# AIM-Harvard/pyradiomics

Hardware: AMD Instinct MI355X
Metric: Mvoxels/s for GLCM+GLRLM build, 512^3 vol @32 bins (higher is better)
Workload: dtype u8 levels / u32 counts / f64 out; 1 GPU; GLCM+GLRLM matrix build, 512^3 int32+uint8 volume resident in HBM, 32 grey levels, full mask, 13 angles, uniform levels; one volume per GPU (batch sharding, no collective); size=512, levels=32, dist=uniform, deferred_mode=pipeline

## Files before the change

pyradiomics_amd/csrc/prad_api.hip:

```cpp
#include "prad_runtime.h"
#include "kernels_generic.h"
#include "kernels_pairs.h"
#include "kernels_sweep.h"
#include "kernels_sweepfw.h"
#include "kernels_sweepfw2.h"
#include "kernels_neigh.h"
#include "kernels_glszm.h"
#include "kernels_voxel.h"
#include "kernels_voxslide.h"
#include "kernels_mcc.h"
#include "kernels_voxtex.h"
#include "prad_sweep_plan.h"
#include "prad_internal.h"

#include <algorithm>
#include <atomic>
#include <chrono>
#include <cmath>
#include <condition_variable>
#include <cstdlib>
#include <deque>
#include <limits>
#include <mutex>
#include <thread>
// ... 366 lines not shown
  for (size_t i = (na & ~(size_t)3) + t; i < na; i += nt) a[i] = 0;
  for (size_t i = t; i < nb; i += nt) b[i] = 0;
  for (size_t i = t; i < nc; i += nt) c3[i] = 0;
}

struct VolState {
  bool valid = false;
  SweepPlan p;
  int Ng = 0, Nr = 0, Na = 0;
  double *glcm = nullptr, *glrlm = nullptr;
  uint8_t *levels = nullptr, *rowzero = nullptr;
  uint8_t *levels16 = nullptr;
  u32 *acc = nullptr, *glcm_acc = nullptr, *glrlm_acc = nullptr;
  int *multi = nullptr;
  int *flags_d = nullptr;
  bool packed_inline = false;
  int lane = -1;
};

bool fin_ride(const SweepKnobs &kn) { return kn.fin_ride; }

struct ZeroNeed {
  u32 *acc = nullptr, *rz = nullptr, *fl = nullptr;
  size_t acc_w = 0, rz_w = 0, fl_w = 0;
};
struct SetZero {
  u32 *rz = nullptr, *fl = nullptr;
  size_t rz_cap = 0;
  size_t rz_used = 0;
  size_t rz_zero = 0;
  bool fl_zero = false;
};
constexpr int kPipeSets = 4;
SetZero *set_zero_book() {
  static thread_local SetZero book[kPipeSets];
  return book;
}
void set_zero_forget() {
  for (int i = 0; i < kPipeSets; i++) set_zero_book()[i] = SetZero();
}
int launch_zero3(hipStream_t s, const ZeroNeed &z) {
  const size_t total_w = z.acc_w + z.rz_w + z.fl_w;
  if (total_w == 0) return PRAD_OK;
  const unsigned gx = (unsigned)std::max<size_t>(1, std::min<size_t>((total_w / 4 + 255) / 256, 1024));
  hipLaunchKernelGGL(zero3_kernel, dim3(gx), dim3(256), 0, s, z.acc, z.acc_w, z.rz, z.rz_w, z.fl, z.fl_w);
  return check_launch("zero3_kernel");
}

int vol_prepare(Call &k, const SweepKnobs &kn, const SweepPlan &p, int Ng, int Nr, double *glcm, double *glrlm, VolState &v,
                ZeroNeed *defer = nullptr) {
  Context &c = *k.c;
  v.lane = c.lane;
  v.valid = true;
  v.p = p;
  v.Ng = Ng;
  v.Nr = Nr;
  v.Na = k.Na;
  v.glcm = glcm;
  v.glrlm = glrlm;
  v.flags_d = k.flags_d;
  const long long nrows = (long long)p.Nz * p.Ny;
  v.levels = nullptr;
  if (!(p.fw2 && p.fw2_rows && p.lines.count > 0 && p.row_slot >= 0)) {
    PRAD_TRY(c.get<uint8_t>("levels", (size_t)nrows * p.pitch + 1024, &v.levels));
    v.levels += 512;
  }
  v.levels16 = nullptr;
  if (p.fw2) {
    PRAD_TRY(c.get<uint8_t>("levels16", (size_t)nrows * p.pitch16 + 4096, &v.levels16));
    v.levels16 += 2048;
  }
  const size_t nglcm = glcm ? (size_t)k.Na * Ng * Ng : 0, nglrlm = glrlm ? (size_t)k.Na * Ng * Nr : 0;
  const size_t nctl = 2 * PRAD_MAX_SWEEP + (size_t)PRAD_FW_WORK_STRIDE * (PRAD_FW_DOMAINS * PRAD_MAX_SWEEP + 1);
  PRAD_TRY(c.get<u32>("sweep_acc", nglcm + nglrlm + nctl, &v.acc));
  v.glcm_acc = v.acc;
  v.glrlm_acc = v.acc + nglcm;
  v.multi = (int *)(v.acc + nglcm + nglrlm);
  v.rowzero = nullptr;
  if (p.fw) PRAD_TRY(c.get<uint8_t>("rowzero", (size_t)nrows + 64, &v.rowzero));
  ZeroNeed z;
  z.acc = v.acc;
  z.acc_w = nglcm + nglrlm + nctl;
  z.rz = reinterpret_cast<u32 *>(v.rowzero);
  z.rz_w = v.rowzero ? ((size_t)nrows + 3) / 4 : 0;
  z.fl = reinterpret_cast<u32 *>(v.flags_d);
  z.fl_w = 4;
  if (c.lane >= 0 && c.lane < kPipeSets) {
    SetZero &S = set_zero_book()[c.lane];
    const size_t cap = v.rowzero ? c.bufs[c.key("rowzero")].cap : 0;
    if (fin_ride(kn)) {
      if (S.rz == z.rz && S.rz_cap == cap && z.rz_w <= S.rz_zero) z.rz_w = 0;
      if (S.fl == z.fl && S.fl_zero) z.fl_w = 0;
    }
    S.rz = z.rz;
    S.rz_cap = cap;
    S.rz_used = v.rowzero ? ((size_t)nrows + 3) / 4 : 0;
    S.rz_zero = 0;
    S.fl = z.fl;
    S.fl_zero = false;
  }
  if (defer) {
    *defer = z;
    return PRAD_OK;
  }
  return launch_zero3(k.s, z);
}

bool pipeline_volume(const SweepPlan &p, bool glcm, bool glrlm) {
  if (!(p.ok && p.lines.count > 0 && glcm && glrlm)) return false;
  return (p.fw && p.fused) || p.fw2;
}
bool pack_inline_ok(const Call &k, const VolState &v) {
  if (!(v.glcm && v.glrlm && v.p.pitch == v.p.Nx && v.p.padw == 0 && (k.g.n % 16) == 0 &&
        ((((uintptr_t)k.image) | ((uintptr_t)k.mask) | ((uintptr_t)v.levels)) & 15) == 0))
    return false;
  if (k.g.n >= (1LL << 31)) return false;
  if (v.p.fw2) return v.levels16 && v.p.pitch16 == 2 * v.p.Nx && (((uintptr_t)v.levels16) & 15) == 0;
  return v.p.fw && v.p.fused;
}

// ... 171 lines not shown
      hipLaunchKernelGGL(finalize_glrlm_kernel, dim3(blocks_for((long long)Ng * Nr * Na)), dim3(256), 0, k.s,
                         v.glrlm_acc, v.multi, Ng, Nr, Na, glrlm, (const int *)v.flags_d, sticky);
      PRAD_TRY(check_launch("finalize_glrlm_kernel"));
      latched = sticky != nullptr;
    }
  }
  if (sticky && !latched) {
    hipLaunchKernelGGL(latch_flags_kernel, dim3(1), dim3(1), 0, k.s, v.flags_d, sticky);
    PRAD_TRY(check_launch("latch_flags_kernel"));
  }
  return PRAD_OK;
}

int sweep_glcm_glrlm(Call &k, const SweepKnobs &kn, const SweepPlan &p, int Ng, int Nr, double *glcm, double *glrlm, bool *used) {
  Context &c = *k.c;
  VolState v;
  PRAD_TRY(vol_prepare(k, kn, p, Ng, Nr, glcm, glrlm, v));
  PRAD_TRY(vol_pack_standalone(k, v));
  PackJob pj;
  memset(&pj, 0, sizeof(pj));
  PRAD_TRY(vol_sweep(k, kn, v, pj));
  int *sticky = nullptr;
  if (c.deferred) PRAD_TRY(c.get<int>("deferred_sticky", 16, &sticky));
  PRAD_TRY(vol_finalize(k, kn, v, sticky));
  if (c.deferred) {
    *used = true;
    return PRAD_OK;
  }
  PRAD_TRY(read_flags(k));
  *used = (k.flags_h[0] == 0 && k.flags_h[2] == 0);
  return PRAD_OK;
}

struct PipeState {
  VolState pending;
  VolState walked;
  hipStream_t s = nullptr;
  unsigned long long seq = 0;
  hipEvent_t ev = nullptr;
  int mode = -1;
};
PipeState &pipe_state() {
  static thread_local PipeState p;
  return p;
}
bool pipeline_mode(const SweepKnobs &kn) {
  PipeState &ps = pipe_state();
  if (ps.mode < 0) ps.mode = kn.lanes_mode ? 0 : 1;
  return ps.mode == 1;
}
int pipeline_sticky(Context &c, int **sticky) { return c.get<int>("deferred_sticky", 16, sticky); }

bool fin_job_empty(const FinJob &fj) { return fj.Na == 0 && fj.zn[0] + fj.zn[1] + fj.zn[2] == 0; }

bool fin_can_ride(const SweepKnobs &kn, const VolState &v) {
  const SweepPlan &p = v.p;
  if (!(v.glcm && v.glrlm && p.fw && p.fused && p.lines.count > 0 && v.levels && v.lane >= 0 && v.lane < kPipeSets)) return false;
  if (p.row_slot >= 0 && p.fw_xblocks == 0) return false;
  if (!finalize_one(kn) || (long long)v.Ng * v.Nr >= (1LL << 30) || v.Ng > 255 || v.Na > PRAD_MAX_SWEEP || v.Na != p.aset.count) return false;
  return ((long long)v.Ng * v.Nr + (long long)v.Ng * v.Ng) * v.Na < (1LL << 31);
}
bool fin_host_ok(const SweepKnobs &kn, const PipeState &ps, const VolState &host, const PackJob &pj, hipStream_t s) {
  const SweepPlan &p = host.p;
  if (!(fin_ride(kn) && ps.s == s && host.glcm && host.glrlm && p.fw && p.fused && p.lines.count > 0)) return false;
  const size_t lds = p.fw_xblocks > 0 ? std::max(p.lds_fw, p.lds_fw_rows) : p.lds_fw;
  return lds >= (size_t)PRAD_FIN_SCRATCH_BYTES && p.fw_blocks >= 1 && p.fw_blocks < 32768;
}

FinJob make_fin_job(const VolState &host, const VolState *walked, const ZeroNeed *need, int new_lane) {
  FinJob j;
  memset(&j, 0, sizeof(j));
  const int nline = host.p.fw_blocks;
  if (walked) {
    const VolState &w = *walked;
    j.Na = w.Na;
    j.Ng = w.Ng;
    j.Nr = w.Nr;
    j.Nz = w.p.Nz;
    j.Ny = w.p.Ny;
    j.Nx = w.p.Nx;
    j.pitch = w.p.pitch;
    j.L = w.levels;
    j.glcm_acc = w.glcm_acc;
    j.glrlm_acc = w.glrlm_acc;
    j.glcm_out = w.glcm;
    j.glrlm_out = w.glrlm;
    j.multi = w.multi;
    j.flags = w.flags_d;
    const FwSet &fs = host.p.fwset;
    for (int a = 0; a < w.Na; a++) {
      for (int d = 0; d < 3; d++) j.off[a][d] = (signed char)w.p.aset.off[a][d];
      const int role = a % fs.count, idx = a / fs.count;
      const int b = (fs.first_block[role] + idx < fs.first_block[role + 1]) ? fs.first_block[role] + idx : a % nline;
      j.ablock[a] = (short)b;
    }
  }
  const int wl = walked ? walked->lane : -1;
  if (need && need->acc_w > 0 && new_lane >= 0 && new_lane < kPipeSets && new_lane != host.lane && new_lane != wl) {
    j.z[0] = need->acc;
    j.zn[0] = (unsigned)need->acc_w;
  }
  if (new_lane >= 0 && new_lane < kPipeSets) {
    const int t = (new_lane + 1) % kPipeSets;
    SetZero &S = set_zero_book()[t];
    if (t != host.lane && t != wl && t != new_lane && S.rz_zero < S.rz_used && S.rz) {
      j.z[1] = S.rz;
      j.zn[1] = (unsigned)S.rz_used;
      S.rz_zero = S.rz_used;
    }
    if (t != host.lane && t != wl && t != new_lane && S.fl && !S.fl_zero) {
      j.z[2] = S.fl;
      j.zn[2] = 4;
      S.fl_zero = true;
    }
  }
  return j;
}

int pipeline_finish_walked(Context &c, const SweepKnobs &kn, hipStream_t s) {
  PipeState &ps = pipe_state();
  if (!ps.walked.valid) return PRAD_OK;
  Call k;
  k.c = &c;
  k.s = s;
  k.Na = ps.walked.Na;
  k.flags_d = ps.walked.flags_d;
  int *sticky = nullptr;
  PRAD_TRY(pipeline_sticky(c, &sticky));
  PRAD_TRY(vol_finalize(k, kn, ps.walked, sticky));
  ps.walked.valid = false;
  return PRAD_OK;
}

int pipeline_retire(Context &c, const SweepKnobs &kn, hipStream_t s, const PackJob &pj, bool keep = false, const ZeroNeed *need = nullptr,
                    int new_lane = -1) {
  PipeState &ps = pipe_state();
  const bool host_ok = fin_host_ok(kn, ps, ps.pending, pj, s);
  if (ps.s != s) {
    if (!ps.ev) PRAD_HIP(hipEventCreateWithFlags(&ps.ev, hipEventDisableTiming));
    PRAD_HIP(hipEventRecord(ps.ev, ps.s));
    PRAD_HIP(hipStreamWaitEvent(s, ps.ev, 0));
  }
  Call k;
  k.c = &c;
  k.s = s;
  k.Na = ps.pending.Na;
  k.flags_d = ps.pending.flags_d;
  int *sticky = nullptr;
  PRAD_TRY(pipeline_sticky(c, &sticky));
  FinJob fj;
  memset(&fj, 0, sizeof(fj));
  if (host_ok) {
    const bool rides = ps.walked.valid && fin_can_ride(kn, ps.walked) && ps.walked.lane != ps.pending.lane && ps.walked.lane != new_lane;
    if (ps.walked.valid && !rides) PRAD_TRY(pipeline_finish_walked(c, kn, s));
    fj = make_fin_job(ps.pending, rides ? &ps.walked : nullptr, need, new_lane);
    fj.sticky = sticky;
    ps.walked.valid = false;
  } else {
    PRAD_TRY(pipeline_finish_walked(c, kn, s));
  }
  if (need && need->acc_w > 0 && fj.zn[0] == 0) {
    ZeroNeed acc;
    acc.acc = need->acc;
    acc.acc_w = need->acc_w;
    PRAD_TRY(launch_zero3(s, acc));
  }
  PRAD_TRY(vol_sweep(k, kn, ps.pending, pj, fj));
  if (keep && fin_ride(kn) && fin_can_ride(kn, ps.pending)) {
    ps.walked = ps.pending;
    ps.pending.valid = false;
    return PRAD_OK;
  }
  PRAD_TRY(vol_finalize(k, kn, ps.pending, sticky));
  ps.pending.valid = false;
  return PRAD_OK;
}

int pipeline_flush(Context &c, const SweepKnobs &kn) {
  PipeState &ps = pipe_state();
  if (!ps.pending.valid && !ps.walked.valid) return PRAD_OK;
  PackJob none;
  memset(&none, 0, sizeof(none));
  const size_t before = c.times.size();
  if (ps.pending.valid) PRAD_TRY(pipeline_retire(c, kn, ps.s, none));
  else PRAD_TRY(pipeline_finish_walked(c, kn, ps.s));
  if (c.timing_accumulate) c.all_times.insert(c.all_times.end(), c.times.begin() + (long)before, c.times.end());
  return PRAD_OK;
}
int pipeline_flush(Context &c) {
  PipeState &ps = pipe_state();
  if (!ps.pending.valid && !ps.walked.valid) return PRAD_OK;
  return pipeline_flush(c, sweep_knobs_from_env());
}

int pipeline_step(Call &k, const SweepKnobs &kn, const SweepPlan &p, int Ng, int Nr, double *glcm, double *glrlm, bool *handled) {
  Context &c = *k.c;
  PipeState &ps = pipe_state();
  *handled = false;
  if (!pipeline_volume(p, glcm != nullptr, glrlm != nullptr)) return pipeline_flush(c, kn);
  VolState v;
  ZeroNeed need;
  PRAD_TRY(vol_prepare(k, kn, p, Ng, Nr, glcm, glrlm, v, &need));
  PackJob pj;
  memset(&pj, 0, sizeof(pj));
  bool inl = false;
  if (ps.pending.valid) {
    inl = pack_inline_ok(k, v) && ps.pending.p.fw2 == v.p.fw2 && !kn.no_inline_pack;
    if (inl) pj = make_pack_job(k, kn, v, &ps.pending);
    const bool ride = fin_host_ok(kn, ps, ps.pending, pj, k.s) && need.acc_w + need.rz_w + need.fl_w < ((size_t)1 << 30);
    ZeroNeed now = need;
    if (ride) {
      now.acc_w = 0;
      need.rz_w = need.fl_w = 0;
    }
    PRAD_TRY(launch_zero3(k.s, now));
    PRAD_TRY(pipeline_retire(c, kn, k.s, pj, true, ride ? &need : nullptr, v.lane));
  } else {
    PRAD_TRY(pipeline_finish_walked(c, kn, ps.s));
    PRAD_TRY(launch_zero3(k.s, need));
  }
  if (!inl) PRAD_TRY(vol_pack_standalone(k, v));
  v.packed_inline = inl;
  ps.pending = v;
  ps.s = k.s;
  *handled = true;
  return PRAD_OK;
}

int pairs_glcm_glrlm(Call &k, const SweepKnobs &kn, int Ng, int Nr, double *glcm, double *glrlm, bool *used) {
  *used = false;
  Context &c = *k.c;
  if (k.vm.voxels || k.g.nd > 3 || Ng < 1 || Ng > PRAD_PAIR_LDS_WORDS || k.Na > PRAD_PAIR_MAXA || k.g.n >= 0x7fffffffLL ||
      kn.no_pairs)
    return PRAD_OK;
  int dims[3] = {1, 1, 1};
  for (int d = 0; d < k.g.nd; d++) dims[3 - k.g.nd + d] = k.g.size[d];
  PairAngles A;
  memset(&A, 0, sizeof(A));
  A.n = k.Na;
  for (int a = 0; a < k.Na; a++)
    for (int d = 0; d < k.g.nd; d++) {
      const int o = k.angles_h[a * k.g.nd + d];
      if (o < -127 || o > 127) return PRAD_OK;
      A.o[a][3 - k.g.nd + d] = (signed char)o;
    }
  if (glrlm && Nr < std::max(dims[0], std::max(dims[1], dims[2]))) return PRAD_OK;
  const size_t gwords = glcm ? (size_t)k.Na * Ng * Ng : 0, rwords = glrlm ? (size_t)k.Na * Ng * Nr : 0;
  if ((gwords + rwords) * sizeof(u32) > ((size_t)1 << 30)) return PRAD_OK;
  hipStream_t s = k.s;
  lev16 *L = nullptr;
  u32 *gacc = nullptr, *racc = nullptr, *counts = nullptr;
  int *multi = nullptr;
  PRAD_TRY(c.get<lev16>("pairs_levels", (size_t)k.g.n + 8, &L));
  if (glcm) PRAD_TRY(c.get<u32>("pairs_glcm_acc", gwords, &gacc));
  if (glrlm) {
    PRAD_TRY(c.get<u32>("pairs_glrlm_acc", rwords, &racc));
    PRAD_TRY(c.get<u32>("pairs_counts", (size_t)Ng, &counts));
// ... 57 lines not shown
    PRAD_TRY(check_launch("pairs_glrlm_kernel"));
    hipLaunchKernelGGL(pairs_multi_check_kernel, dim3(gx, (unsigned)k.Na), dim3(256), 0, s, A, L, dims[0], dims[1], dims[2], multi, k.flags_d);
    PRAD_TRY(check_launch("pairs_multi_check_kernel"));
    hipLaunchKernelGGL(pairs_run1_kernel, dim3((unsigned)((Ng * k.Na + 3) / 4)), dim3(256), 0, s, racc, counts, Ng, Nr, k.Na, k.flags_d);
    PRAD_TRY(check_launch("pairs_run1_kernel"));
    const long long total = (long long)Ng * Nr * k.Na;
    hipLaunchKernelGGL(finalize_glrlm_kernel, dim3(blocks_for(total)), dim3(256), 0, s, racc, multi, Ng, Nr, k.Na, glrlm,
                       (const int *)nullptr, (int *)nullptr);
    PRAD_TRY(check_launch("finalize_glrlm_kernel"));
  }
  PRAD_TRY(read_flags(k));
  *used = k.flags_h[0] == 0;
  if (!*used) {
    PRAD_HIP(hipMemsetAsync(k.flags_d, 0, sizeof(int) * 4, s));
  }
  return PRAD_OK;
}

}
namespace prad {
int texture_pairs_runs(const int32_t *image, const uint8_t *mask, const int *size, int Nd, const int *angles,
                       int Na, int Ng, int Nr, int Nvox, const int *voxels, int kernelRadius, int force2Ddim,
                       double *glcm, double *glrlm, hipStream_t s) {
  if (!glcm && !glrlm) return fail(PRAD_E_ARG, "both outputs are NULL");
  if (Ng < 1 || (glrlm && Nr < 1)) return fail(PRAD_E_ARG, "Ng/Nr must be >= 1");
  Context &c = ctx();
  PRAD_TRY(c.ensure_device());
  const SweepKnobs kn = sweep_knobs_from_env();
  struct LaneGuard {
    Context &c;
    ~LaneGuard() { c.lane = -1; }
  } lane_guard{c};
  bool pipe = c.deferred && !voxels && pipeline_mode(kn);
  if (c.deferred && !voxels && !pipe) {
    PRAD_TRY(c.lane_begin(s, &s));
    if (c.lane >= 0) c.lane += kPipeSets;
  }
  if (pipe) c.lane = (int)(pipe_state().seq++ % (unsigned)kPipeSets);
  Call k;
  PRAD_TRY(setup_call(k, image, mask, size, Nd, angles, Na, Nvox, voxels, kernelRadius, force2Ddim, s, false));
  SweepPlan p = plan_sweep(k, kn, Ng, Nr, glcm != nullptr, glrlm != nullptr);
  if (pipe && !pipeline_volume(p, glcm != nullptr, glrlm != nullptr)) {
    const hipStream_t user = s;
    PRAD_TRY(pipeline_flush(c, kn));
    pipe = false;
    c.lane = -1;
    PRAD_TRY(c.lane_begin(user, &s));
    if (c.lane >= 0) c.lane += kPipeSets;
    PRAD_TRY(setup_call(k, image, mask, size, Nd, angles, Na, Nvox, voxels, kernelRadius, force2Ddim, s, false));
    p = plan_sweep(k, kn, Ng, Nr, glcm != nullptr, glrlm != nullptr);
  }
  PRAD_TRY(c.begin_call(s));
  if (!p.ok) PRAD_HIP(hipMemsetAsync(k.flags_d, 0, sizeof(int) * 4, s));
  bool done = false;
  c.last_variant = !p.ok ? "none" : (p.fw2 ? "fw2" : (p.fw && glcm && glrlm ? "fw" : "lines"));
  if (pipe) {
    PRAD_TRY(pipeline_step(k, kn, p, Ng, Nr, glcm, glrlm, &done));
    if (done) c.last_path = "sweep";
  }
  if (!done && p.ok) {
    PRAD_TRY(sweep_glcm_glrlm(k, kn, p, Ng, Nr, glcm, glrlm, &done));
    if (done) c.last_path = "sweep";
  }
  if (!done && !c.deferred) {
    PRAD_TRY(pairs_glcm_glrlm(k, kn, Ng, Nr, glcm, glrlm, &done));
    if (done) {
      c.last_path = "pairs";
      c.last_variant = "pairs";
    }
  }
  if (!done) {
    if (glcm) PRAD_TRY(generic_glcm(k, Ng, glcm));
    if (glrlm) PRAD_TRY(generic_glrlm(k, Ng, Nr, glrlm));
    PRAD_TRY(read_flags(k));
    c.last_path = "generic";
  }
  PRAD_TRY(c.end_call(s));
  if (c.deferred && done) return PRAD_OK;
  PRAD_HIP(hipStreamSynchronize(s));
  return k.flags_h[1] ? PRAD_INDEX_ERROR : PRAD_OK;
}
}
namespace {

int pairs_neigh(Call &k, bool ngtdm, int Ng, int alpha, double *out, bool *used, bool box_only = false) {
  *used = false;
  Context &c = *k.c;
  if (k.vm.voxels || k.g.nd > 3 || Ng < 1 || Ng > 65535 || k.g.n >= 0x7fffffffLL || getenv("PRAD_NO_PAIRS")) return PRAD_OK;
  int dims[3] = {1, 1, 1};
  for (int d = 0; d < k.g.nd; d++) dims[3 - k.g.nd + d] = k.g.size[d];
// ... 460 lines not shown
}

namespace prad {
int zone_features_launch(Context &c, hipStream_t s, const double *P, int Ni, int Njcap, long long stride_i,
                         const double *jvals_d, const int *nj_dev, double *out_d, int *empty_d);
}
extern "C" {

const char *prad_version(void) { return kVersion; }
const char *prad_last_error(void) { return err_state().msg; }
const char *prad_last_path(void) { return ctx().last_path; }
const char *prad_last_variant(void) { return ctx().last_variant; }
#ifdef PRAD_FW_STAMPS
int prad_debug_fw_stamps(unsigned long long *out, int slot, int nwaves) {
  if (!out || nwaves < 1 || nwaves > 8192 || slot < 0 || slot > 1) return PRAD_E_ARG;
  PRAD_HIP(hipDeviceSynchronize());
  PRAD_HIP(hipMemcpyFromSymbol(out, HIP_SYMBOL(prad::prad_fw_stamps), sizeof(unsigned long long) * prad::FP_COUNT * (size_t)nwaves,
                               sizeof(unsigned long long) * prad::FP_COUNT * 8192 * (size_t)slot));
  return PRAD_OK;
}
#endif

int prad_device_count(void) {
  int n = 0;
  if (hipGetDeviceCount(&n) != hipSuccess) return 0;
  return n;
}

int prad_set_device(int device) {
  int n = prad_device_count();
  if (device < 0 || device >= n) return fail(PRAD_E_ARG, "device %d not in [0,%d)", device, n);
  Context &c = ctx();
  if (c.device != device) {
    if ((pipe_state().pending.valid || pipe_state().walked.valid) && c.device_set && hipSetDevice(c.device) == hipSuccess) {
      (void)pipeline_flush(c);
      if (pipe_state().s) (void)hipStreamSynchronize(pipe_state().s);
    }
    pipe_state().pending.valid = false;
    pipe_state().walked.valid = false;
    set_zero_forget();
    pipe_state().s = nullptr;
    pipe_state().ev = nullptr;
    c.own_stream = nullptr;
    for (int l = 0; l < PRAD_MAX_LANES; l++) {
      if (c.lane_stream[l]) (void)hipStreamSynchronize(c.lane_stream[l]);
      c.lane_stream[l] = nullptr;
      c.lane_in[l] = nullptr;
    }
    c.event_pool.clear();
    c.events_used = 0;
  }
  c.device = device;
  c.device_set = true;
  PRAD_HIP(hipSetDevice(device));
  return PRAD_OK;
}
int prad_get_device(void) { return ctx().device; }

long long prad_workspace_bytes(void) {
  long long total = 0;
  for (const auto &kv : ctx().bufs) total += (long long)kv.second.cap;
  return total;
}
int prad_release_workspace(void) {
  Context &c = ctx();
  if (pipe_state().pending.valid || pipe_state().walked.valid) {
    (void)pipeline_flush(c);
    if (pipe_state().s) (void)hipStreamSynchronize(pipe_state().s);
    pipe_state().pending.valid = false;
    pipe_state().walked.valid = false;
  }
  set_zero_forget();
  glszm_state().valid = false;
  for (auto &kv : c.bufs) {
    if (kv.second.p) (void)hipFree(kv.second.p);
    kv.second.p = nullptr;
    kv.second.cap = 0;
  }
  (void)hipDeviceSynchronize();
  for (auto &kv : c.pinned) {
    if (kv.second.p) (void)hipHostFree(kv.second.p);
    kv.second.p = nullptr;
    kv.second.cap = 0;
  }
  c.bufs.clear();
  c.pinned.clear();
  if (c.arena) (void)hipHostFree(c.arena);
  c.arena = nullptr;
  c.arena_pos = 0;
  release_image_queues();
  c.angles_cached.clear();
  c.tables_cached.clear();
  StageRing &r = stage_ring();
  for (int i = 0; i < kStageRing; i++) {
    r.buf[i] = nullptr;
    r.busy[i] = false;
  }
  return PRAD_OK;
}

int prad_timing_begin(void) {
  Context &c = ctx();
  c.timing_only.clear();
// ... 29 lines not shown
  Context &c = ctx();
  double total = 0;
  if (!family) {
    for (auto &ab : c.all_calls) {
      float ms = 0;
      if (hipEventSynchronize(ab.second) != hipSuccess || hipEventElapsedTime(&ms, ab.first, ab.second) != hipSuccess) return -1.0;
      total += ms;
    }
    return total;
  }
  for (auto &t : c.all_times) {
    if (t.family != family) continue;
    float ms = 0;
    if (hipEventSynchronize(t.b) != hipSuccess || hipEventElapsedTime(&ms, t.a, t.b) != hipSuccess) return -1.0;
    total += ms;
  }
  return total;
}

int prad_set_deferred(int on) {
  Context &c = ctx();
  if (c.ensure_device() != PRAD_OK) return PRAD_E_HIP;
  if (on && !c.has("deferred_sticky")) {
    int *sticky = nullptr;
    PRAD_TRY(c.get<int>("deferred_sticky", 16, &sticky));
    PRAD_HIP(hipMemset(sticky, 0, sizeof(int) * 16));
  }
  c.deferred = on != 0;
  return PRAD_OK;
}
int prad_set_lanes(int n) {
  Context &c = ctx();
  if (n < 0 || n > PRAD_MAX_LANES) return fail(PRAD_E_ARG, "lanes=%d outside [0, %d]", n, PRAD_MAX_LANES);
  PRAD_TRY(c.lanes_sync());
  c.lanes = n;
  c.lane_seq = 0;
  return PRAD_OK;
}
int prad_set_deferred_mode(int mode) {
  if (mode < -1 || mode > 1) return fail(PRAD_E_ARG, "deferred mode %d (0 lanes, 1 pipeline, -1 environment default)", mode);
  Context &c = ctx();
  PRAD_TRY(c.ensure_device());
  PipeState &ps = pipe_state();
  PRAD_TRY(pipeline_flush(c));
  if (ps.s) PRAD_HIP(hipStreamSynchronize(ps.s));
  PRAD_TRY(c.lanes_sync());
  ps.mode = mode;
  return PRAD_OK;
}
int prad_set_workspace(int id) {
  if (id < 0 || id > 7) return fail(PRAD_E_ARG, "workspace %d outside [0, 7]", id);
  ctx().workspace = id;
  return PRAD_OK;
}
int prad_result_alloc(size_t bytes, void **out) {
  if (!out) return fail(PRAD_E_ARG, "result_alloc: out is NULL");
  Context &c = ctx();
  PRAD_TRY(c.ensure_device());
  return c.arena_alloc(bytes, out);
}
int prad_deferred_join(void *stream) {
  Context &c = ctx();
  PRAD_TRY(c.ensure_device());
  PipeState &ps = pipe_state();
  PRAD_TRY(pipeline_flush(c));
  if (ps.s && ps.s != (hipStream_t)stream) {
    if (!ps.ev) PRAD_HIP(hipEventCreateWithFlags(&ps.ev, hipEventDisableTiming));
    PRAD_HIP(hipEventRecord(ps.ev, ps.s));
    PRAD_HIP(hipStreamWaitEvent((hipStream_t)stream, ps.ev, 0));
  }
  return c.lanes_join((hipStream_t)stream);
}
int prad_deferred_mark(int *flag, void *stream) {
  Context &c = ctx();
  PRAD_TRY(c.ensure_device());
  if (!flag || !c.in_arena(flag, sizeof(int))) return fail(PRAD_E_ARG, "deferred_mark: flag must lie in the result arena");
  PRAD_TRY(pipeline_flush(c));
  int *sticky = nullptr;
  PRAD_TRY(c.get<int>("deferred_sticky", 16, &sticky));
  PRAD_HIP(hipMemcpyAsync(flag, sticky, sizeof(int), hipMemcpyDeviceToHost, (hipStream_t)stream));
  return PRAD_OK;
}
int prad_deferred_status(void *stream) {
  Context &c = ctx();
  PRAD_TRY(c.ensure_device());
  PRAD_TRY(pipeline_flush(c));
  if (pipe_state().s) PRAD_HIP(hipStreamSynchronize(pipe_state().s));
  PRAD_HIP(hipStreamSynchronize((hipStream_t)stream));
  PRAD_TRY(c.lanes_sync());
  if (!c.has("deferred_sticky")) return PRAD_OK;
  int *sticky = nullptr;
  PRAD_TRY(c.get<int>("deferred_sticky", 16, &sticky));
  void *pin = nullptr;
  PRAD_TRY(c.get_pinned("sticky_h", 64, &pin));
  PRAD_HIP(hipMemcpyAsync(pin, sticky, sizeof(int), hipMemcpyDeviceToHost, (hipStream_t)stream));
  PRAD_HIP(hipStreamSynchronize((hipStream_t)stream));
  const int h = *(const int *)pin;
  if (h) {
    PRAD_HIP(hipMemsetAsync(sticky, 0, sizeof(int), (hipStream_t)stream));
    PRAD_HIP(hipStreamSynchronize((hipStream_t)stream));
    return fail(PRAD_E_DEFERRED, "a deferred GLCM/GLRLM call saw masked levels outside [1, Ng]; repeat it synchronously");
  }
  return PRAD_OK;
}

double prad_last_device_ms(void) {
  Context &c = ctx();
  if (!c.call_timed) return -1.0;
  float ms = 0;
  if (hipEventElapsedTime(&ms, c.call_a, c.call_b) != hipSuccess) return -1.0;
  return ms;
}

double prad_last_kernel_ms(const char *family) {
  Context &c = ctx();
  double total = 0;
  bool any = false;
  for (auto &t : c.times) {
    if (family && t.family != family) continue;
    float ms = 0;
// ... 410 lines not shown
```

pyradiomics_amd/csrc/prad_runtime.h:

```cpp
#pragma once

#include <hip/hip_runtime.h>
#include <stdint.h>
#include <stdio.h>
#include <stdarg.h>
#include <string.h>
#include <stdlib.h>
#include <string>
#include <vector>
#include <map>

#include "../../include/pyradiomics_amd.h"

namespace prad {

struct ErrorState {
  char msg[512];
  ErrorState() { msg[0] = 0; }
};
inline ErrorState &err_state() {
  static thread_local ErrorState e;
  return e;
}
inline int fail(int code, const char *fmt, ...) {
// ... 63 lines not shown

  int ensure_device() {
    if (!device_set) {
      int n = 0;
      hipError_t e = hipGetDeviceCount(&n);
      if (e != hipSuccess || n <= 0)
        return fail(PRAD_E_HIP, "no HIP device visible (hipGetDeviceCount: %s) -- this library has no CPU fallback",
                    hipGetErrorString(e));
      device_set = true;
    }
    PRAD_HIP(hipSetDevice(device));
    if (!own_stream) PRAD_HIP(hipStreamCreateWithFlags(&own_stream, hipStreamNonBlocking));
    return PRAD_OK;
  }

  std::string key(const char *name) const {
    std::string k(name);
    if (k.compare(0, 9, "deferred_") != 0) {
      if (lane >= 0) k += "#" + std::to_string(lane);
      if (workspace) k += "~" + std::to_string(workspace);
    }
    return k + "@" + std::to_string(device);
  }
  bool has(const char *name) const { return bufs.find(key(name)) != bufs.end(); }
  std::vector<int> &angle_cache() { return angles_cached[key("angles")]; }
  int lane_begin(hipStream_t user, hipStream_t *s) {
    if (lanes == 0) {
      const char *e = getenv("PRAD_LANES");
      lanes = e ? atoi(e) : 2;
      lanes = lanes < 1 ? 1 : (lanes > PRAD_MAX_LANES ? PRAD_MAX_LANES : lanes);
    }
    if (lanes == 1) return PRAD_OK;
    const int l = (int)(lane_seq++ % (unsigned)lanes);
    if (!lane_stream[l]) {
      PRAD_HIP(hipStreamCreateWithFlags(&lane_stream[l], hipStreamNonBlocking));
      PRAD_HIP(hipEventCreateWithFlags(&lane_in[l], hipEventDisableTiming));
    }
    PRAD_HIP(hipEventRecord(lane_in[l], user));
    PRAD_HIP(hipStreamWaitEvent(lane_stream[l], lane_in[l], 0));
    lane = l;
    *s = lane_stream[l];
    return PRAD_OK;
  }
  int lanes_join(hipStream_t s) {
    for (int l = 0; l < PRAD_MAX_LANES; l++)
      if (lane_stream[l]) {
        PRAD_HIP(hipEventRecord(lane_in[l], lane_stream[l]));
        PRAD_HIP(hipStreamWaitEvent(s, lane_in[l], 0));
      }
    return PRAD_OK;
  }
  int lanes_sync() {
    for (int l = 0; l < PRAD_MAX_LANES; l++)
      if (lane_stream[l]) PRAD_HIP(hipStreamSynchronize(lane_stream[l]));
    return PRAD_OK;
  }

  int get(const char *name, size_t bytes, void **out) {
    DevBuf &b = bufs[key(name)];
    if (b.cap < bytes) {
      if (b.p) (void)hipFree(b.p);
      b.p = nullptr;
      b.cap = 0;
      size_t want = bytes + bytes / 8 + 256;
      hipError_t e = hipMalloc(&b.p, want);
      if (e != hipSuccess) {
        b.p = nullptr;
        return fail(PRAD_E_NOMEM, "hipMalloc(%zu) for workspace '%s' failed: %s", want, name, hipGetErrorString(e));
      }
      b.cap = want;
    }
    *out = b.p;
    return PRAD_OK;
  }
// ... 206 lines not shown
```

pyradiomics_amd/csrc/prad_sweep_plan.h:

```cpp
#pragma once
#include "kernels_sweepfw2.h"

#include <algorithm>
#include <cstdlib>
#include <cstring>

namespace prad {
#pragma GCC visibility push(hidden)

struct Knob {
  bool set = false;
  long long v = 0;
};
struct SweepKnobs {
  bool no_fw = false;
  bool no_fw2 = false;
  bool no_fw2_rows = false;
  bool fw2_noskip1 = false;
  bool fw_xrole_off = false;
  Knob threads, lpl, lines_blocks;
  Knob fw2_copies, fw2_rs, fw2_rows_waves;
  Knob fw_budget_kb, fw_rs, fw_blocks, fw_threads, fw_per_wave, fw_cl, fw_xcd;
  Knob fw_rows_threads, fw_xblocks, fw_xgpd;
  Knob pack_every;
  bool fin_ride = true;
  bool finalize_one = true;
  bool no_inline_pack = false;
  bool no_pairs = false;
  bool lanes_mode = false;
};

inline Knob env_knob(const char *name, bool wide = false) {
  Knob k;
  if (const char *e = getenv(name)) {
    k.set = true;
    k.v = wide ? atoll(e) : (long long)atoi(e);
  }
  return k;
}
inline bool env_not_zero(const char *name) {
  const char *e = getenv(name);
  return !(e && atoi(e) == 0 && e[0] != '\0');
}

inline SweepKnobs sweep_knobs_from_env() {
  SweepKnobs k;
  k.no_fw = getenv("PRAD_NO_FW") != nullptr;
  k.no_fw2 = getenv("PRAD_NO_FW2") != nullptr;
  k.no_fw2_rows = getenv("PRAD_NO_FW2_ROWS") != nullptr;
  k.fw2_noskip1 = getenv("PRAD_FW2_NOSKIP1") != nullptr;
  {
    const char *e = getenv("PRAD_FW_XROLE");
    k.fw_xrole_off = e && atoi(e) == 0;
  }
  k.threads = env_knob("PRAD_THREADS");
  k.lpl = env_knob("PRAD_LPL");
  k.lines_blocks = env_knob("PRAD_LINES_BLOCKS");
  k.fw2_copies = env_knob("PRAD_FW2_COPIES");
  k.fw2_rs = env_knob("PRAD_FW2_RS", true);
  k.fw2_rows_waves = env_knob("PRAD_FW2_ROWS_WAVES");
  k.fw_budget_kb = env_knob("PRAD_FW_BUDGET_KB");
  k.fw_rs = env_knob("PRAD_FW_RS");
  k.fw_blocks = env_knob("PRAD_FW_BLOCKS");
  k.fw_threads = env_knob("PRAD_FW_THREADS");
  k.fw_per_wave = env_knob("PRAD_FW_PER_WAVE");
  k.fw_cl = env_knob("PRAD_FW_CL");
  k.fw_xcd = env_knob("PRAD_FW_XCD");
  k.fw_rows_threads = env_knob("PRAD_FW_ROWS_THREADS");
  k.fw_xblocks = env_knob("PRAD_FW_XBLOCKS", true);
  k.fw_xgpd = env_knob("PRAD_FW_XGPD");
  k.pack_every = env_knob("PRAD_PACK_EVERY");
  k.fin_ride = env_not_zero("PRAD_FIN_RIDE");
  k.finalize_one = env_not_zero("PRAD_FINALIZE_ONE");
  k.no_inline_pack = getenv("PRAD_NO_INLINE_PACK") != nullptr;
  k.no_pairs = getenv("PRAD_NO_PAIRS") != nullptr;
  {
    const char *e = getenv("PRAD_DEFERRED_MODE");
    k.lanes_mode = e && strcmp(e, "lanes") == 0;
  }
  return k;
}

struct SweepPlan {
  bool ok = false;
  int Nz = 1, Ny = 1, Nx = 1;
  SweepSet lines;
  int row_slot = -1;
  bool skip1 = false;
  bool fused = false;
  int LPL = 1;
  int pitch = 0, padw = 0;
  bool vec_rows = false;
  AngleSet aset;
  int RS = 0;
  bool LONG = false;
  int threads = 256;
  size_t lds_bytes = 0;
  int RSr = 0;
  bool LONGr = false;
  size_t lds_bytes_rows = 0;
  bool fw = false;
  int fwK = 8;
  int fw_blocks = 1;
  int fw_threads = 1024;
  int fw_rows_threads = 512;
  int RSfw = 0;
  bool LONGfw = false;
  size_t lds_fw = 0;
  int RSfw_rows = 0;
  size_t lds_fw_rows = 0;
  int fw_xblocks = 0;
// ... 316 lines not shown
```

Before: 297,400 Mvoxels/s.

## Run two deferred pipelines on alternating streams for large volumes

Splits the single deferred pipeline state into two instances, each owning its own set of lanes and zero books. Large volumes (at least 2^27 voxels, which includes 512^3) alternate between two non-blocking streams so consecutive volumes' sweep and finalize work can overlap on the GPU. Output address ranges are tracked so that overlapping outputs force a flush and ordering between the pipelines. The cost is more bookkeeping, extra events and cross-stream waits, and a risk of resource contention or ordering bugs.

New measurement: 314,700 Mvoxels/s (median of 6 runs). +5.8%, better.

```diff
diff --git a/pyradiomics_amd/csrc/prad_api.hip b/pyradiomics_amd/csrc/prad_api.hip
--- a/pyradiomics_amd/csrc/prad_api.hip
+++ b/pyradiomics_amd/csrc/prad_api.hip
@@ -422,12 +422,16 @@
   bool fl_zero = false;
 };
 constexpr int kPipeSets = 4;
+constexpr int kPipes = 2;
+constexpr int kAllPipeSets = kPipes * kPipeSets;
+inline bool pipe_set(int lane) { return lane >= 0 && lane < kAllPipeSets; }
+inline int next_pipe_set(int lane) { return lane - lane % kPipeSets + (lane + 1) % kPipeSets; }
 SetZero *set_zero_book() {
-  static thread_local SetZero book[kPipeSets];
+  static thread_local SetZero book[kAllPipeSets];
   return book;
 }
 void set_zero_forget() {
-  for (int i = 0; i < kPipeSets; i++) set_zero_book()[i] = SetZero();
+  for (int i = 0; i < kAllPipeSets; i++) set_zero_book()[i] = SetZero();
 }
 int launch_zero3(hipStream_t s, const ZeroNeed &z) {
   const size_t total_w = z.acc_w + z.rz_w + z.fl_w;
@@ -475,7 +479,7 @@
   z.rz_w = v.rowzero ? ((size_t)nrows + 3) / 4 : 0;
   z.fl = reinterpret_cast<u32 *>(v.flags_d);
   z.fl_w = 4;
-  if (c.lane >= 0 && c.lane < kPipeSets) {
+  if (pipe_set(c.lane)) {
     SetZero &S = set_zero_book()[c.lane];
     const size_t cap = v.rowzero ? c.bufs[c.key("rowzero")].cap : 0;
     if (fin_ride(kn)) {
@@ -713,30 +717,81 @@
   return PRAD_OK;
 }
 
+constexpr long long kTwinMinVoxels = 1LL << 27;
+struct OutRange {
+  const char *lo, *hi;
+};
 struct PipeState {
   VolState pending;
   VolState walked;
   hipStream_t s = nullptr;
   unsigned long long seq = 0;
   hipEvent_t ev = nullptr;
+  int base = 0;
+  std::vector<OutRange> outs;
+};
+struct PipeShared {
   int mode = -1;
+  unsigned long long twin_calls = 0;
 };
-PipeState &pipe_state() {
-  static thread_local PipeState p;
+PipeState &pipe_state(int i) {
+  static thread_local PipeState p[kPipes];
+  p[i].base = i * kPipeSets;
+  return p[i];
+}
+PipeShared &pipe_shared() {
+  static thread_local PipeShared p;
   return p;
 }
 bool pipeline_mode(const SweepKnobs &kn) {
-  PipeState &ps = pipe_state();
+  PipeShared &ps = pipe_shared();
   if (ps.mode < 0) ps.mode = kn.lanes_mode ? 0 : 1;
   return ps.mode == 1;
 }
+bool pipelines_busy() {
+  for (int i = 0; i < kPipes; i++)
+    if (pipe_state(i).pending.valid || pipe_state(i).walked.valid) return true;
+  return false;
+}
+int pipeline_order(PipeState &ps, hipStream_t s) {
+  if (!ps.s || ps.s == s) return PRAD_OK;
+  if (!ps.ev) PRAD_HIP(hipEventCreateWithFlags(&ps.ev, hipEventDisableTiming));
+  PRAD_HIP(hipEventRecord(ps.ev, ps.s));
+  PRAD_HIP(hipStreamWaitEvent(s, ps.ev, 0));
+  return PRAD_OK;
+}
+void out_ranges_add(PipeState &ps, const double *glcm, size_t nglcm, const double *glrlm, size_t nglrlm) {
+  const OutRange r[2] = {{(const char *)glcm, (const char *)(glcm + nglcm)}, {(const char *)glrlm, (const char *)(glrlm + nglrlm)}};
+  for (int i = 0; i < 2; i++) {
+    if (!r[i].lo) continue;
+    bool known = false;
+    for (OutRange &o : ps.outs)
+      if (o.lo <= r[i].lo && r[i].hi <= o.hi) known = true;
+    if (known) continue;
+    if (ps.outs.size() >= 64) {
+      for (const OutRange &o : ps.outs) {
+        ps.outs[0].lo = std::min(ps.outs[0].lo, o.lo);
+        ps.outs[0].hi = std::max(ps.outs[0].hi, o.hi);
+      }
+      ps.outs.resize(1);
+    }
+    ps.outs.push_back(r[i]);
+  }
+}
+bool out_ranges_overlap(const PipeState &ps, const double *glcm, size_t nglcm, const double *glrlm, size_t nglrlm) {
+  const OutRange r[2] = {{(const char *)glcm, (const char *)(glcm + nglcm)}, {(const char *)glrlm, (const char *)(glrlm + nglrlm)}};
+  for (int i = 0; i < 2; i++)
+    for (const OutRange &o : ps.outs)
+      if (r[i].lo && r[i].lo < o.hi && o.lo < r[i].hi) return true;
+  return false;
+}
 int pipeline_sticky(Context &c, int **sticky) { return c.get<int>("deferred_sticky", 16, sticky); }
 
 bool fin_job_empty(const FinJob &fj) { return fj.Na == 0 && fj.zn[0] + fj.zn[1] + fj.zn[2] == 0; }
 
 bool fin_can_ride(const SweepKnobs &kn, const VolState &v) {
   const SweepPlan &p = v.p;
-  if (!(v.glcm && v.glrlm && p.fw && p.fused && p.lines.count > 0 && v.levels && v.lane >= 0 && v.lane < kPipeSets)) return false;
+  if (!(v.glcm && v.glrlm && p.fw && p.fused && p.lines.count > 0 && v.levels && pipe_set(v.lane))) return false;
   if (p.row_slot >= 0 && p.fw_xblocks == 0) return false;
   if (!finalize_one(kn) || (long long)v.Ng * v.Nr >= (1LL << 30) || v.Ng > 255 || v.Na > PRAD_MAX_SWEEP || v.Na != p.aset.count) return false;
   return ((long long)v.Ng * v.Nr + (long long)v.Ng * v.Ng) * v.Na < (1LL << 31);
@@ -748,7 +803,7 @@
   return lds >= (size_t)PRAD_FIN_SCRATCH_BYTES && p.fw_blocks >= 1 && p.fw_blocks < 32768;
 }
 
-FinJob make_fin_job(const VolState &host, const VolState *walked, const ZeroNeed *need, int new_lane) {
+FinJob make_fin_job(const PipeState &ps, const VolState &host, const VolState *walked, const ZeroNeed *need, int new_lane) {
   FinJob j;
   memset(&j, 0, sizeof(j));
   const int nline = host.p.fw_blocks;
@@ -777,12 +832,13 @@
     }
   }
   const int wl = walked ? walked->lane : -1;
-  if (need && need->acc_w > 0 && new_lane >= 0 && new_lane < kPipeSets && new_lane != host.lane && new_lane != wl) {
+  const bool mine = new_lane >= ps.base && new_lane < ps.base + kPipeSets;
+  if (need && need->acc_w > 0 && mine && new_lane != host.lane && new_lane != wl) {
     j.z[0] = need->acc;
     j.zn[0] = (unsigned)need->acc_w;
   }
-  if (new_lane >= 0 && new_lane < kPipeSets) {
-    const int t = (new_lane + 1) % kPipeSets;
+  if (mine) {
+    const int t = next_pipe_set(new_lane);
     SetZero &S = set_zero_book()[t];
     if (t != host.lane && t != wl && t != new_lane && S.rz_zero < S.rz_used && S.rz) {
       j.z[1] = S.rz;
@@ -798,8 +854,7 @@
   return j;
 }
 
-int pipeline_finish_walked(Context &c, const SweepKnobs &kn, hipStream_t s) {
-  PipeState &ps = pipe_state();
+int pipeline_finish_walked(Context &c, const SweepKnobs &kn, PipeState &ps, hipStream_t s) {
   if (!ps.walked.valid) return PRAD_OK;
   Call k;
   k.c = &c;
@@ -813,15 +868,10 @@
   return PRAD_OK;
 }
 
-int pipeline_retire(Context &c, const SweepKnobs &kn, hipStream_t s, const PackJob &pj, bool keep = false, const ZeroNeed *need = nullptr,
-                    int new_lane = -1) {
-  PipeState &ps = pipe_state();
+int pipeline_retire(Context &c, const SweepKnobs &kn, PipeState &ps, hipStream_t s, const PackJob &pj, bool keep = false,
+                    const ZeroNeed *need = nullptr, int new_lane = -1) {
   const bool host_ok = fin_host_ok(kn, ps, ps.pending, pj, s);
-  if (ps.s != s) {
-    if (!ps.ev) PRAD_HIP(hipEventCreateWithFlags(&ps.ev, hipEventDisableTiming));
-    PRAD_HIP(hipEventRecord(ps.ev, ps.s));
-    PRAD_HIP(hipStreamWaitEvent(s, ps.ev, 0));
-  }
+  PRAD_TRY(pipeline_order(ps, s));
   Call k;
   k.c = &c;
   k.s = s;
@@ -833,12 +883,12 @@
   memset(&fj, 0, sizeof(fj));
   if (host_ok) {
     const bool rides = ps.walked.valid && fin_can_ride(kn, ps.walked) && ps.walked.lane != ps.pending.lane && ps.walked.lane != new_lane;
-    if (ps.walked.valid && !rides) PRAD_TRY(pipeline_finish_walked(c, kn, s));
-    fj = make_fin_job(ps.pending, rides ? &ps.walked : nullptr, need, new_lane);
+    if (ps.walked.valid && !rides) PRAD_TRY(pipeline_finish_walked(c, kn, ps, s));
+    fj = make_fin_job(ps, ps.pending, rides ? &ps.walked : nullptr, need, new_lane);
     fj.sticky = sticky;
     ps.walked.valid = false;
   } else {
-    PRAD_TRY(pipeline_finish_walked(c, kn, s));
+    PRAD_TRY(pipeline_finish_walked(c, kn, ps, s));
   }
   if (need && need->acc_w > 0 && fj.zn[0] == 0) {
     ZeroNeed acc;
@@ -857,28 +907,47 @@
   return PRAD_OK;
 }
 
-int pipeline_flush(Context &c, const SweepKnobs &kn) {
-  PipeState &ps = pipe_state();
+int pipeline_flush(Context &c, const SweepKnobs &kn, PipeState &ps) {
   if (!ps.pending.valid && !ps.walked.valid) return PRAD_OK;
   PackJob none;
   memset(&none, 0, sizeof(none));
   const size_t before = c.times.size();
-  if (ps.pending.valid) PRAD_TRY(pipeline_retire(c, kn, ps.s, none));
-  else PRAD_TRY(pipeline_finish_walked(c, kn, ps.s));
+  const int rc = ps.pending.valid ? pipeline_retire(c, kn, ps, ps.s, none) : pipeline_finish_walked(c, kn, ps, ps.s);
+  if (rc != PRAD_OK) ps.pending.valid = ps.walked.valid = false;
   if (c.timing_accumulate) c.all_times.insert(c.all_times.end(), c.times.begin() + (long)before, c.times.end());
-  return PRAD_OK;
+  return rc;
+}
+int pipeline_flush(Context &c, const SweepKnobs &kn) {
+  int rc = PRAD_OK;
+  for (int i = 0; i < kPipes; i++) {
+    const int r = pipeline_flush(c, kn, pipe_state(i));
+    if (rc == PRAD_OK) rc = r;
+  }
+  return rc;
 }
 int pipeline_flush(Context &c) {
-  PipeState &ps = pipe_state();
-  if (!ps.pending.valid && !ps.walked.valid) return PRAD_OK;
+  if (!pipelines_busy()) return PRAD_OK;
   return pipeline_flush(c, sweep_knobs_from_env());
 }
-
-int pipeline_step(Call &k, const SweepKnobs &kn, const SweepPlan &p, int Ng, int Nr, double *glcm, double *glrlm, bool *handled) {
+int pipelines_order(hipStream_t s) {
+  for (int i = 0; i < kPipes; i++) PRAD_TRY(pipeline_order(pipe_state(i), s));
+  return PRAD_OK;
+}
+int pipelines_sync() {
+  for (int i = 0; i < kPipes; i++) {
+    PipeState &ps = pipe_state(i);
+    if (ps.s) PRAD_HIP(hipStreamSynchronize(ps.s));
+    ps.outs.clear();
+  }
+  return PRAD_OK;
+}
+
+int pipeline_step(Call &k, const SweepKnobs &kn, PipeState &ps, const SweepPlan &p, int Ng, int Nr, double *glcm, double *glrlm,
+                  bool *handled) {
   Context &c = *k.c;
-  PipeState &ps = pipe_state();
   *handled = false;
   if (!pipeline_volume(p, glcm != nullptr, glrlm != nullptr)) return pipeline_flush(c, kn);
+  PRAD_TRY(pipeline_order(ps, k.s));
   VolState v;
   ZeroNeed need;
   PRAD_TRY(vol_prepare(k, kn, p, Ng, Nr, glcm, glrlm, v, &need));
@@ -895,15 +964,16 @@
       need.rz_w = need.fl_w = 0;
     }
     PRAD_TRY(launch_zero3(k.s, now));
-    PRAD_TRY(pipeline_retire(c, kn, k.s, pj, true, ride ? &need : nullptr, v.lane));
+    PRAD_TRY(pipeline_retire(c, kn, ps, k.s, pj, true, ride ? &need : nullptr, v.lane));
   } else {
-    PRAD_TRY(pipeline_finish_walked(c, kn, ps.s));
+    PRAD_TRY(pipeline_finish_walked(c, kn, ps, ps.s));
     PRAD_TRY(launch_zero3(k.s, need));
   }
   if (!inl) PRAD_TRY(vol_pack_standalone(k, v));
   v.packed_inline = inl;
   ps.pending = v;
   ps.s = k.s;
+  out_ranges_add(ps, glcm, (size_t)k.Na * Ng * Ng, glrlm, (size_t)k.Na * Ng * Nr);
   *handled = true;
   return PRAD_OK;
 }
@@ -1027,21 +1097,46 @@
     ~LaneGuard() { c.lane = -1; }
   } lane_guard{c};
   bool pipe = c.deferred && !voxels && pipeline_mode(kn);
+  const hipStream_t user = s;
   if (c.deferred && !voxels && !pipe) {
     PRAD_TRY(c.lane_begin(s, &s));
-    if (c.lane >= 0) c.lane += kPipeSets;
-  }
-  if (pipe) c.lane = (int)(pipe_state().seq++ % (unsigned)kPipeSets);
+    if (c.lane >= 0) c.lane += kAllPipeSets;
+  }
+  int inst = 0;
+  if (pipe) {
+    bool twin = kn.pipe_twin == 1;
+    if (kn.pipe_twin < 0 && size && Nd >= 1 && Nd <= PRAD_MAX_ND) {
+      long long n = 1;
+      for (int d = 0; d < Nd; d++) n *= std::max(size[d], 1);
+      twin = n >= kTwinMinVoxels;
+    }
+    if (twin) {
+      inst = (int)(pipe_shared().twin_calls++ % (unsigned)kPipes);
+      PRAD_TRY(c.twin_streams());
+      PRAD_TRY(c.lane_enter(inst, user, &s));
+    } else {
+      PRAD_TRY(pipeline_flush(c, kn, pipe_state(1)));
+    }
+    PipeState &other = pipe_state(1 - inst);
+    if (Na >= 1 && out_ranges_overlap(other, glcm, glcm ? (size_t)Na * Ng * Ng : 0, glrlm, glrlm ? (size_t)Na * Ng * Nr : 0)) {
+      PRAD_TRY(pipeline_flush(c, kn, other));
+      PRAD_TRY(pipeline_order(other, s));
+      other.outs.clear();
+    }
+    PipeState &ps = pipe_state(inst);
+    c.lane = ps.base + (int)(ps.seq++ % (unsigned)kPipeSets);
+  }
   Call k;
   PRAD_TRY(setup_call(k, image, mask, size, Nd, angles, Na, Nvox, voxels, kernelRadius, force2Ddim, s, false));
   SweepPlan p = plan_sweep(k, kn, Ng, Nr, glcm != nullptr, glrlm != nullptr);
   if (pipe && !pipeline_volume(p, glcm != nullptr, glrlm != nullptr)) {
-    const hipStream_t user = s;
     PRAD_TRY(pipeline_flush(c, kn));
+    PRAD_TRY(pipelines_order(user));
     pipe = false;
     c.lane = -1;
+    s = user;
     PRAD_TRY(c.lane_begin(user, &s));
-    if (c.lane >= 0) c.lane += kPipeSets;
+    if (c.lane >= 0) c.lane += kAllPipeSets;
     PRAD_TRY(setup_call(k, image, mask, size, Nd, angles, Na, Nvox, voxels, kernelRadius, force2Ddim, s, false));
     p = plan_sweep(k, kn, Ng, Nr, glcm != nullptr, glrlm != nullptr);
   }
@@ -1050,7 +1145,7 @@
   bool done = false;
   c.last_variant = !p.ok ? "none" : (p.fw2 ? "fw2" : (p.fw && glcm && glrlm ? "fw" : "lines"));
   if (pipe) {
-    PRAD_TRY(pipeline_step(k, kn, p, Ng, Nr, glcm, glrlm, &done));
+    PRAD_TRY(pipeline_step(k, kn, pipe_state(inst), p, Ng, Nr, glcm, glrlm, &done));
     if (done) c.last_path = "sweep";
   }
   if (!done && p.ok) {
@@ -1577,15 +1672,19 @@
   if (device < 0 || device >= n) return fail(PRAD_E_ARG, "device %d not in [0,%d)", device, n);
   Context &c = ctx();
   if (c.device != device) {
-    if ((pipe_state().pending.valid || pipe_state().walked.valid) && c.device_set && hipSetDevice(c.device) == hipSuccess) {
+    if (pipelines_busy() && c.device_set && hipSetDevice(c.device) == hipSuccess) {
       (void)pipeline_flush(c);
-      if (pipe_state().s) (void)hipStreamSynchronize(pipe_state().s);
-    }
-    pipe_state().pending.valid = false;
-    pipe_state().walked.valid = false;
+      (void)pipelines_sync();
+    }
+    for (int i = 0; i < kPipes; i++) {
+      PipeState &ps = pipe_state(i);
+      ps.pending.valid = false;
+      ps.walked.valid = false;
+      ps.s = nullptr;
+      ps.ev = nullptr;
+      ps.outs.clear();
+    }
     set_zero_forget();
-    pipe_state().s = nullptr;
-    pipe_state().ev = nullptr;
     c.own_stream = nullptr;
     for (int l = 0; l < PRAD_MAX_LANES; l++) {
       if (c.lane_stream[l]) (void)hipStreamSynchronize(c.lane_stream[l]);
@@ -1609,11 +1708,10 @@
 }
 int prad_release_workspace(void) {
   Context &c = ctx();
-  if (pipe_state().pending.valid || pipe_state().walked.valid) {
+  if (pipelines_busy()) {
     (void)pipeline_flush(c);
-    if (pipe_state().s) (void)hipStreamSynchronize(pipe_state().s);
-    pipe_state().pending.valid = false;
-    pipe_state().walked.valid = false;
+    (void)pipelines_sync();
+    for (int i = 0; i < kPipes; i++) pipe_state(i).pending.valid = pipe_state(i).walked.valid = false;
   }
   set_zero_forget();
   glszm_state().valid = false;
@@ -1709,6 +1807,11 @@
 int prad_set_lanes(int n) {
   Context &c = ctx();
   if (n < 0 || n > PRAD_MAX_LANES) return fail(PRAD_E_ARG, "lanes=%d outside [0, %d]", n, PRAD_MAX_LANES);
+  if (pipelines_busy()) {
+    PRAD_TRY(c.ensure_device());
+    PRAD_TRY(pipeline_flush(c));
+    PRAD_TRY(pipelines_sync());
+  }
   PRAD_TRY(c.lanes_sync());
   c.lanes = n;
   c.lane_seq = 0;
@@ -1718,11 +1821,10 @@
   if (mode < -1 || mode > 1) return fail(PRAD_E_ARG, "deferred mode %d (0 lanes, 1 pipeline, -1 environment default)", mode);
   Context &c = ctx();
   PRAD_TRY(c.ensure_device());
-  PipeState &ps = pipe_state();
   PRAD_TRY(pipeline_flush(c));
-  if (ps.s) PRAD_HIP(hipStreamSynchronize(ps.s));
+  PRAD_TRY(pipelines_sync());
   PRAD_TRY(c.lanes_sync());
-  ps.mode = mode;
+  pipe_shared().mode = mode;
   return PRAD_OK;
 }
 int prad_set_workspace(int id) {
@@ -1739,13 +1841,8 @@
 int prad_deferred_join(void *stream) {
   Context &c = ctx();
   PRAD_TRY(c.ensure_device());
-  PipeState &ps = pipe_state();
   PRAD_TRY(pipeline_flush(c));
-  if (ps.s && ps.s != (hipStream_t)stream) {
-    if (!ps.ev) PRAD_HIP(hipEventCreateWithFlags(&ps.ev, hipEventDisableTiming));
-    PRAD_HIP(hipEventRecord(ps.ev, ps.s));
-    PRAD_HIP(hipStreamWaitEvent((hipStream_t)stream, ps.ev, 0));
-  }
+  PRAD_TRY(pipelines_order((hipStream_t)stream));
   return c.lanes_join((hipStream_t)stream);
 }
 int prad_deferred_mark(int *flag, void *stream) {
@@ -1753,6 +1850,7 @@
   PRAD_TRY(c.ensure_device());
   if (!flag || !c.in_arena(flag, sizeof(int))) return fail(PRAD_E_ARG, "deferred_mark: flag must lie in the result arena");
   PRAD_TRY(pipeline_flush(c));
+  PRAD_TRY(pipelines_order((hipStream_t)stream));
   int *sticky = nullptr;
   PRAD_TRY(c.get<int>("deferred_sticky", 16, &sticky));
   PRAD_HIP(hipMemcpyAsync(flag, sticky, sizeof(int), hipMemcpyDeviceToHost, (hipStream_t)stream));
@@ -1762,7 +1860,7 @@
   Context &c = ctx();
   PRAD_TRY(c.ensure_device());
   PRAD_TRY(pipeline_flush(c));
-  if (pipe_state().s) PRAD_HIP(hipStreamSynchronize(pipe_state().s));
+  PRAD_TRY(pipelines_sync());
   PRAD_HIP(hipStreamSynchronize((hipStream_t)stream));
   PRAD_TRY(c.lanes_sync());
   if (!c.has("deferred_sticky")) return PRAD_OK;
diff --git a/pyradiomics_amd/csrc/prad_runtime.h b/pyradiomics_amd/csrc/prad_runtime.h
--- a/pyradiomics_amd/csrc/prad_runtime.h
+++ b/pyradiomics_amd/csrc/prad_runtime.h
@@ -119,14 +119,26 @@
     }
     if (lanes == 1) return PRAD_OK;
     const int l = (int)(lane_seq++ % (unsigned)lanes);
+    const int rc = lane_enter(l, user, s);
+    if (rc == PRAD_OK) lane = l;
+    return rc;
+  }
+  int lane_enter(int l, hipStream_t user, hipStream_t *s) {
     if (!lane_stream[l]) {
       PRAD_HIP(hipStreamCreateWithFlags(&lane_stream[l], hipStreamNonBlocking));
       PRAD_HIP(hipEventCreateWithFlags(&lane_in[l], hipEventDisableTiming));
     }
     PRAD_HIP(hipEventRecord(lane_in[l], user));
     PRAD_HIP(hipStreamWaitEvent(lane_stream[l], lane_in[l], 0));
-    lane = l;
     *s = lane_stream[l];
+    return PRAD_OK;
+  }
+  int twin_streams() {
+    for (int l = 0; l < 2; l++)
+      if (!lane_stream[l]) {
+        PRAD_HIP(hipStreamCreateWithFlags(&lane_stream[l], hipStreamNonBlocking));
+        PRAD_HIP(hipEventCreateWithFlags(&lane_in[l], hipEventDisableTiming));
+      }
     return PRAD_OK;
   }
   int lanes_join(hipStream_t s) {
diff --git a/pyradiomics_amd/csrc/prad_sweep_plan.h b/pyradiomics_amd/csrc/prad_sweep_plan.h
--- a/pyradiomics_amd/csrc/prad_sweep_plan.h
+++ b/pyradiomics_amd/csrc/prad_sweep_plan.h
@@ -28,6 +28,7 @@
   bool no_inline_pack = false;
   bool no_pairs = false;
   bool lanes_mode = false;
+  int pipe_twin = -1;
 };
 
 inline Knob env_knob(const char *name, bool wide = false) {
@@ -77,6 +78,10 @@
   {
     const char *e = getenv("PRAD_DEFERRED_MODE");
     k.lanes_mode = e && strcmp(e, "lanes") == 0;
+  }
+  {
+    const char *e = getenv("PRAD_PIPE_TWIN");
+    k.pipe_twin = (e && e[0] != '\0') ? (atoi(e) != 0 ? 1 : 0) : -1;
   }
   return k;
 }
```
